# aleksandrina-streltsova/lidar-global-registration

Hardware: AMD Instinct MI355X
Metric: scan-pair registrations/sec (higher is better)
Workload: dtype f32

## Files before the change

### lidar-global-registration_amd/csrc/lgr_align.hip

```cpp
#include <rocprim/device/device_scan.hpp>

#include <chrono>
#include <cmath>

#include <climits>

#include "lgr_cloud.h"
#include "lgr_host.h"

namespace {

__device__ __forceinline__ float corr_threshold(float a, float b, float dthr) {
    float m = (a < b) ? b : a;
    return (dthr < m) ? dthr : m;
}

template <int KMAX>
__device__ __forceinline__ float cluster_distance(int i, int j, int k, const int32_t* __restrict__ knn_a, const int32_t* __restrict__ knn_b,
                                                   const int32_t* __restrict__ ab_idx) {
    int nb[KMAX];
#pragma unroll
    for (int b = 0; b < KMAX; ++b) nb[b] = b < k ? knn_b[(size_t) j * k + b] : -2;
    int consistent = 0, pairs = 0;
    for (int a0 = 0; a0 < k; a0 += 8) {
// ... 107 lines not shown
    size_t tb = 0;
    LGR_HIP(ctx, rocprim::exclusive_scan(nullptr, tb, flags, pos, 0, (size_t) ns, rocprim::plus<int>(), ctx->stream));
    void* tmp;
    LGR_TRY(lgr_ws(ctx, WS_GRID_TMP, tb, &tmp));
    LGR_HIP(ctx, rocprim::exclusive_scan(tmp, tb, flags, pos, 0, (size_t) ns, rocprim::plus<int>(), ctx->stream));
    filter_emit<<<cdiv(ns, 256), 256, 0, ctx->stream>>>(ns, d_ij_idx, flags, pos, dist, thr_s, thr_t, distance_thr, d_out);
    int* h;
    LGR_TRY(lgr_pinned(ctx, 64, (void**) &h));
    LGR_HIP(ctx, hipMemcpyAsync(h, pos + (ns - 1), 4, hipMemcpyDeviceToHost, ctx->stream));
    LGR_HIP(ctx, hipMemcpyAsync(h + 1, flags + (ns - 1), 4, hipMemcpyDeviceToHost, ctx->stream));
    LGR_HIP(ctx, hipStreamSynchronize(ctx->stream));
    *n_out = h[0] + h[1];
    LGR_HIP(ctx, hipGetLastError());
    return LGR_OK;
}

static void tick(lgr_ctx* ctx, int i) { (void) hipEventRecord(ctx->ev[i], ctx->stream); }

__global__ void gather_rows12_kernel(const float* __restrict__ pts, const int32_t* __restrict__ idx, int m, float* __restrict__ out) {
    size_t e = (size_t) blockIdx.x * blockDim.x + threadIdx.x;
    if (e >= (size_t) m * 12) return;
    out[e] = pts[(size_t) idx[e / 12] * 12 + e % 12];
}
static void gather_rows12(lgr_ctx* ctx, const float* pts, const int32_t* idx, int m, float* out) {
    gather_rows12_kernel<<<cdiv((long long) m * 12, 256), 256, 0, ctx->stream>>>(pts, idx, m, out);
}
__global__ void finalize_kernel(lgr_corr* __restrict__ corr, int n, const int32_t* __restrict__ ks, const int32_t* __restrict__ kt) {
    int i = blockIdx.x * blockDim.x + threadIdx.x;
    if (i >= n) return;
    corr[i].index_query = ks[corr[i].index_query];
    corr[i].index_match = kt[corr[i].index_match];
}

typedef int (*FeatureStage)(lgr_ctx* ctx, const float* kps, int m, const float* surf, int n, float radius, float* out, const lgr_params* p, const float* vp);
struct Descriptor {
    int len;
    FeatureStage stage;
    bool dense;
    int lrf;
};
static int fpfh_stage(lgr_ctx* ctx, const float* kps, int m, const float* surf, int n, float radius, float* out, const lgr_params*, const float*) { return lgr_fpfh_dev(ctx, kps, m, surf, n, radius, out); }
static int shot_stage(lgr_ctx* ctx, const float* kps, int m, const float* surf, int n, float radius, float* out, const lgr_params*, const float*) { return lgr_shot_dev(ctx, kps, m, surf, n, radius, nullptr, out, nullptr); }
static int rops_stage(lgr_ctx* ctx, const float* kps, int m, const float* surf, int n, float radius, float* out, const lgr_params* p, const float* vp) {
    float* kn;
    LGR_TRY(lgr_ws_t(ctx, WS_ROPS_KPS, (size_t) m * 12, &kn));
    LGR_HIP(ctx, hipMemcpyAsync(kn, kps, (size_t) m * 48, hipMemcpyDeviceToDevice, ctx->stream));
    LGR_TRY(lgr_normals_knn_dev(ctx, kn, m, surf, n, p->normal_nr_points, vp, 1));
    return lgr_rops_gravity_dev(ctx, kn, m, surf, n, radius, out);
}
static const Descriptor DESCRIPTORS[] = {
     {33, fpfh_stage, false, LGR_LRF_DEFAULT},
     {352, shot_stage, true, LGR_LRF_DEFAULT},
     {135, rops_stage, true, LGR_LRF_GRAVITY},
};
static_assert(LGR_DESCRIPTOR_FPFH == 0 && LGR_DESCRIPTOR_SHOT == 1 && LGR_DESCRIPTOR_ROPS == 2, "DESCRIPTORS is indexed by descriptor_id");

extern "C" void lgr_default_feature_params(lgr_feature_params* f) {
    if (!f) return;
    memset(f, 0, sizeof(*f));
    f->descriptor_id = LGR_DESCRIPTOR_FPFH;
    f->lrf_id = LGR_LRF_DEFAULT;
}

static int feature_descriptor(lgr_ctx* ctx, const lgr_params* p, const lgr_feature_params* f, const Descriptor** out) {
    *out = &DESCRIPTORS[LGR_DESCRIPTOR_FPFH];
    if (!f) return LGR_OK;
    LGR_CHECK(ctx, f->descriptor_id >= 0 && f->descriptor_id < (int) (sizeof DESCRIPTORS / sizeof *DESCRIPTORS), LGR_ERR_UNSUPPORTED);
    const Descriptor& d = DESCRIPTORS[f->descriptor_id];
    if (d.dense) {
        LGR_CHECK(ctx, f->lrf_id == LGR_LRF_DEFAULT || f->lrf_id == LGR_LRF_GRAVITY || f->lrf_id == LGR_LRF_GT, LGR_ERR_INVALID_ARG);
        LGR_CHECK(ctx, f->lrf_id == d.lrf, LGR_ERR_UNSUPPORTED);
        LGR_CHECK(ctx, p->use_bfmatcher && !p->has_guess, LGR_ERR_UNSUPPORTED);
        LGR_CHECK(ctx, ctx->opt.arithmetic != LGR_ARITH_PCL, LGR_ERR_UNSUPPORTED);
    }
    *out = &d;
    return LGR_OK;
// ... 13 lines not shown
    bool empty = false;
    float *feat[2], *surf[2], *dij, *dji;
    int32_t *ij, *ji;
    FilterTables ftab;
    int ratio_k = 0;
    float ms[3] = {0, 0, 0};
    struct Tables {
        CorrCall* c;
        int operator()(lgr_ctx* cx) const {
            LGR_TRY(filter_cloud_tables(cx, c->kclouds[0], c->ksizes[0], c->p->cluster_k, c->ftab.thr_s, c->ftab.knn_s));
            return filter_cloud_tables(cx, c->kclouds[1], c->ksizes[1], c->p->cluster_k, c->ftab.thr_t, c->ftab.knn_t);
        }
    } tables{this};
    lgr_helper_guard tables_guard;
    struct PrepGuard { lgr_ctx* c; ~PrepGuard() { lgr_match_prepare_cancel(c); } } prep_guard;

    CorrCall(lgr_ctx* ctx, const float* d_src, int ns, const float* d_tgt, int nt, const lgr_params* p, lgr_corr* d_out, int* n_out)
        : ctx(ctx), p(p), clouds{d_src, d_tgt}, kclouds{d_src, d_tgt}, sizes{ns, nt}, ksizes{ns, nt}, d_out(d_out), n_out(n_out), prep_guard{ctx} {}
    CorrCall(const CorrCall&) = delete;
    const float* vp(int side) const { return side == 0 ? (p->has_vp_src ? p->vp_src : nullptr) : (p->has_vp_tgt ? p->vp_tgt : nullptr); }
    float iss_radius(int side) const { return side == 0 ? p->iss_radius_src : p->iss_radius_tgt; }
    bool ratio() const { return p->matching_id == LGR_MATCH_RATIO; }
    bool both_dirs() const { return p->matching_id != LGR_MATCH_ONE_SIDED && !ratio(); }
    template <class T>
    int result(int side, int slot, size_t count, T** out) const { return own[side] ? lgr_cloud_alloc_t(ctx, own[side], count, out) : lgr_ws_t(ctx, slot, count, out); }
};

static int level_features(lgr_ctx* cx, const CorrCall& c, int side, const float* in, int n_in, float voxel, float radius, float* surf,
                          const float* kps, int m, const int32_t* d_list, float* sub, float* out, float* ms, int* nd) {
    const lgr_params* p = c.p;
    tick(cx, 0);
    LGR_TRY(lgr_downsample_dev(cx, in, n_in, voxel, surf, nd));
    tick(cx, 1);
    LGR_TRY(lgr_normals_knn_dev(cx, surf, *nd, nullptr, 0, p->normal_nr_points, c.vp(side), p->normals_available));
    tick(cx, 2);
    if (m) {
        if (d_list) { gather_rows12(cx, kps, d_list, m, sub); kps = sub; }
        LGR_TRY(c.d->stage(cx, kps, m, surf, *nd, radius, out, p, c.vp(side)));
    }
    tick(cx, 3);
    LGR_HIP(cx, hipEventSynchronize(cx->ev[3]));
    float t;
    for (int s = 0; s < 3; ++s) { (void) hipEventElapsedTime(&t, cx->ev[s], cx->ev[s + 1]); ms[s] += t; }
    return LGR_OK;
}

static int ms_initialize(CorrCall& c, int side, MsSide& st) {
    lgr_ctx* ctx = c.ctx;
    const lgr_params* p = c.p;
    const int D = c.d->len, n = c.sizes[side], n_kps = c.ksizes[side];
    const float *d_pcd = c.clouds[side], *d_kps = c.kclouds[side];
    const int k = 5;
    LGR_CHECK(ctx, n >= k, LGR_ERR_INVALID_ARG);
    int32_t* d_nn;
    float* d_d2;
    LGR_TRY(lgr_ws_t(ctx, WS_MS_KNN_I, (size_t) n_kps * k, &d_nn));
    LGR_TRY(lgr_ws_t(ctx, WS_MS_KNN_D, (size_t) n_kps * k, &d_d2));
    LGR_TRY(lgr_knn_dev(ctx, d_kps, n_kps, d_pcd, n, k, d_nn, d_d2));
    std::vector<float> d2((size_t) n_kps * k);
    LGR_HIP(ctx, hipMemcpyAsync(d2.data(), d_d2, d2.size() * 4, hipMemcpyDeviceToHost, ctx->stream));
    LGR_HIP(ctx, hipStreamSynchronize(ctx->stream));
    std::vector<int> level(n_kps);
    for (int i = 0; i < n_kps; ++i) {
        float density = sqrtf(d2[(size_t) i * k + (k - 1)]);
        float feature_radius = sqrtf((float) p->feature_nr_points * density * density / M_PI);
        level[i] = (int) std::floor(std::log2(feature_radius) / std::log2(p->scale_factor));
        st.min_l2 = std::min(level[i], st.min_l2);
        st.max_l2 = std::max(level[i], st.max_l2);
    }
    LGR_CHECK(ctx, (long long) st.max_l2 - st.min_l2 < 64, LGR_ERR_INVALID_ARG);
    std::vector<int> count(st.max_l2 - st.min_l2 + 1, 0);
// ... 704 lines not shown
```

### lidar-global-registration_amd/csrc/lgr_features.hip

```cpp
#include <rocprim/device/device_radix_sort.hpp>
#include <rocprim/device/device_scan.hpp>

#include <algorithm>
#include <cmath>
#include <type_traits>
#include <vector>

#include "lgr_grid.cuh"
#include "lgr_host.h"
#include "lgr_knn_wave.cuh"
#include "lgr_seqsum.h"
#include "lgr_math.cuh"
#include "lgr_libm.cuh"

namespace {

__global__ void voxel_keys(const float* __restrict__ pts, int n, float bx, float by, float bz, float voxel,
                           unsigned long long* __restrict__ keys, int* __restrict__ vals, int* __restrict__ bad) {
    int i = blockIdx.x * blockDim.x + threadIdx.x;
    if (i >= n) return;
    float x = pts[(size_t) i * 12], y = pts[(size_t) i * 12 + 1], z = pts[(size_t) i * 12 + 2];
    unsigned long long k = ~0ull;
    if (lgr_finite3(x, y, z)) {
        int ix = (int) floorf((x - bx) / voxel), iy = (int) floorf((y - by) / voxel), iz = (int) floorf((z - bz) / voxel);
// ... 10 lines not shown
    flags[i] = (k != ~0ull && (i == 0 || keys[i - 1] != k)) ? 1 : 0;
}

__global__ void voxel_accumulate(const float* __restrict__ pts, const unsigned long long* __restrict__ keys,
                                 const int* __restrict__ vals, const int* __restrict__ flags,
                                 const int* __restrict__ rank , int n,
                                 float* __restrict__ out, unsigned long long* __restrict__ out_keys, int* __restrict__ out_first) {
    int i = blockIdx.x * blockDim.x + threadIdx.x;
    if (i >= n || !flags[i]) return;
    unsigned long long k = keys[i];
    float sx = 0.f, sy = 0.f, sz = 0.f, sw = 0.f, snx = 0.f, sny = 0.f, snz = 0.f;
    for (int j = i; j < n && keys[j] == k; ++j) {
        const float4* p = reinterpret_cast<const float4*>(pts + (size_t) vals[j] * 12);
        float4 a = p[0], b = p[1], c = p[2];
        float w = c.x;
        sx += w * a.x; sy += w * a.y; sz += w * a.z;
        sw += w;
        snx += w * b.x; sny += w * b.y; snz += w * b.z;
    }
    float ax = snx / sw, ay = sny / sw, az = snz / sw;
    float norm = __builtin_sqrtf(ax * ax + ay * ay + az * az);
    norm = ((double) norm < 1e-5) ? 1.f : norm;
    int r = rank[i];
    float4* o = reinterpret_cast<float4*>(out + (size_t) r * 12);
    o[0] = make_float4(sx / sw, sy / sw, sz / sw, 1.f);
    o[1] = make_float4(ax / norm, ay / norm, az / norm, 0.f);
    o[2] = make_float4(sw, 0.f, 0.f, 0.f);
    if (out_keys) { out_keys[r] = k; out_first[r] = vals[i]; }
}

constexpr int NB = 128;

template <class IndexOf>
__device__ __forceinline__ void normals_finish(float* __restrict__ p, float px, float py, float pz, int count, IndexOf&& index_of,
                                               const float* __restrict__ surf, float vpx, float vpy, float vpz) {
    const float nanv = __uint_as_float(0x7fc00000u);
    if (count < 3) { p[4] = nanv; p[5] = nanv; p[6] = nanv; p[9] = nanv; return; }
    const float* K = surf + (size_t) index_of(0) * 12;
    float Kx = K[0], Ky = K[1], Kz = K[2];
    float a0 = 0.f, a1 = 0.f, a2 = 0.f, a3 = 0.f, a4 = 0.f, a5 = 0.f, a6 = 0.f, a7 = 0.f, a8 = 0.f;
    for (int j = 0; j < count; ++j) {
        const float* q = surf + (size_t) index_of(j) * 12;
        float x = q[0] - Kx, y = q[1] - Ky, z = q[2] - Kz;
        a0 += x * x; a1 += x * y; a2 += x * z; a3 += y * y; a4 += y * z; a5 += z * z;
        a6 += x; a7 += y; a8 += z;
    }
    float fn = (float) count;
    a0 /= fn; a1 /= fn; a2 /= fn; a3 /= fn; a4 /= fn; a5 /= fn; a6 /= fn; a7 /= fn; a8 /= fn;
    float C[9];
    C[0] = a0 - a6 * a6; C[1] = a1 - a6 * a7; C[2] = a2 - a6 * a8;
    C[4] = a3 - a7 * a7; C[5] = a4 - a7 * a8; C[8] = a5 - a8 * a8;
    C[3] = C[1]; C[6] = C[2]; C[7] = C[5];
    float lambda_min, nx, ny, nz;
    lgr_pcl_eigen33(C, lambda_min, nx, ny, nz);
    float eig_sum = C[0] + C[4] + C[8];
    float curv = (eig_sum != 0.f) ? fabsf(lambda_min / eig_sum) : 0.f;
    float dx = vpx - px, dy = vpy - py, dz = vpz - pz;
    float cos_theta = (dx * nx + dy * ny + dz * nz);
    if (cos_theta < 0.f) { nx = -nx; ny = -ny; nz = -nz; }
    if (lgr_finite3(nx, ny, nz)) {
        float norm = __builtin_sqrtf(nx * nx + ny * ny + nz * nz);
        nx /= norm; ny /= norm; nz /= norm;
    }
    p[4] = nx; p[5] = ny; p[6] = nz; p[9] = curv;
}

__global__ __launch_bounds__(NB) void normals_kernel(GridDev g, const float* __restrict__ surf, float* __restrict__ pts, int n,
                                                      int k, float vpx, float vpy, float vpz, int by_grid) {
    extern __shared__ float smem[];
    float* sd = smem;
    int* si = (int*) (smem + (size_t) k * NB);
    int i = blockIdx.x * NB + threadIdx.x;
    if (by_grid == 1) {
        i = lgr_xcd_tile(blockIdx.x, cdiv_dev(g.n, NB)) * NB + threadIdx.x;
        if (i >= g.n) return;
        i = __float_as_int(g.pxyz[i].w);
    } else if (i >= n) return;
    float* p = pts + (size_t) i * 12;
    float px = p[0], py = p[1], pz = p[2];
    if (by_grid == 2 && lgr_finite3(px, py, pz)) return;
    KnnList<NB> L;
    L.init(sd, si, k, threadIdx.x);
    if (lgr_finite3(px, py, pz) && g.n > 0) lgr_knn_query(g, px, py, pz, L);
    normals_finish(p, px, py, pz, L.count, [&](int j) { return L.index(j); }, surf, vpx, vpy, vpz);
}

constexpr int NW_WAVES = 4;
template <int KPL>
__global__ __launch_bounds__(64 * NW_WAVES) void normals_wave_kernel(GridDev g, const float* __restrict__ surf, float* __restrict__ pts, int k,
                                                                      float vpx, float vpy, float vpz, float r2_init) {
    extern __shared__ int slist[];
    __shared__ unsigned long long sbuf[NW_WAVES][WaveKnn<KPL>::BUF];
    __shared__ int srow[NW_WAVES][128];
    const int lane = threadIdx.x & 63, wv = threadIdx.x >> 6;
    const int n_tiles = cdiv_dev(g.n, 64 * NW_WAVES);
    const int tile = lgr_xcd_tile(blockIdx.x, n_tiles);
    if (tile >= n_tiles) return;
    const int t = (tile * NW_WAVES + wv) * 64 + lane;
    int* list = slist + (size_t) wv * k * 64;
    int qi = -1;
    float px = 0.f, py = 0.f, pz = 0.f;
    if (t < g.n) {
        const float4 q = g.pxyz[t];
        qi = __float_as_int(q.w); px = q.x; py = q.y; pz = q.z;
    }
    float guess = r2_init;
    int count = 0;
    lgr_wave_knn_tile<KPL>(g, qi >= 0, px, py, pz, k, guess, sbuf[wv], srow[wv], [&](int l, const WaveKnn<KPL>& W) {
        const int mk = min(W.m, k);
#pragma unroll
        for (int j = 0; j < KPL; ++j)
            if (W.rank[j] < mk) list[W.rank[j] * 64 + l] = (int) (unsigned) W.key[j];
        if (lane == l) count = mk;
    });
    __builtin_amdgcn_fence(__ATOMIC_RELEASE, "wavefront");
    __builtin_amdgcn_wave_barrier();
    if (qi < 0) return;
    normals_finish(pts + (size_t) qi * 12, px, py, pz, count, [&](int j) { return list[j * 64 + lane]; }, surf, vpx, vpy, vpz);
}

__device__ __forceinline__ float dot3e(float ax, float ay, float az, float bx, float by, float bz) {
    return (ax * bx + az * bz) + ay * by;
}

__device__ __forceinline__ bool pair_features(float p1x, float p1y, float p1z, float n1x, float n1y, float n1z,
                                              float p2x, float p2y, float p2z, float n2x, float n2y, float n2z,
                                              float& f1, float& f2, float& f3) {
    float dx = p2x - p1x, dy = p2y - p1y, dz = p2z - p1z;
    float f4 = __builtin_sqrtf(dot3e(dx, dy, dz, dx, dy, dz));
    if (f4 == 0.0f) return false;
    float angle1 = dot3e(n1x, n1y, n1z, dx, dy, dz) / f4;
    float angle2 = dot3e(n2x, n2y, n2z, dx, dy, dz) / f4;
    float ux = n1x, uy = n1y, uz = n1z, mx = n2x, my = n2y, mz = n2z;
    float a1 = fabsf(angle1), a2 = fabsf(angle2);
    if (lgr_glibc::acosf_(a1) > lgr_glibc::acosf_(a2)) {
        ux = n2x; uy = n2y; uz = n2z; mx = n1x; my = n1y; mz = n1z;
        dx = -dx; dy = -dy; dz = -dz;
        f3 = -angle2;
    } else {
        f3 = angle1;
    }
    float vx = dy * uz - dz * uy, vy = dz * ux - dx * uz, vz = dx * uy - dy * ux;
    float v_norm = __builtin_sqrtf(dot3e(vx, vy, vz, vx, vy, vz));
    if (v_norm == 0.0f) return false;
    vx /= v_norm; vy /= v_norm; vz /= v_norm;
    float wx = uy * vz - uz * vy, wy = uz * vx - ux * vz, wz = ux * vy - uy * vx;
    f2 = dot3e(vx, vy, vz, mx, my, mz);
    float yy = dot3e(wx, wy, wz, mx, my, mz), xx = dot3e(ux, uy, uz, mx, my, mz);
    f1 = lgr_glibc::atan2f_(yy, xx);
    return true;
}
// ... 773 lines not shown
            case 2: r = lgr_glibc::atan2f_(x, b[i]); break;
            case 3: r = lgr_glibc::sinf_(x); break;
            default: r = lgr_glibc::cosf_(x); break;
        }
        out[i] = r;
    }
}
extern "C" int lgr_selfcheck_libm(lgr_ctx* ctx, int fn, const float* a, const float* b, long long n, float* out) {
    lgr_turn turn__(ctx);
    if (!ctx) return LGR_ERR_INVALID_ARG;
    LGR_CHECK(ctx, fn >= 0 && fn <= 6 && a && out && n >= 0 && (fn != 2 || b), LGR_ERR_INVALID_ARG);
    if (n == 0) return LGR_OK;
    float *da, *db, *dout;
    lgr_host_call hc(ctx);
    LGR_TRY(hc.in(a, (size_t) n, &da));
    LGR_TRY(hc.in(fn == 2 ? b : nullptr, (size_t) n, &db));
    LGR_TRY(hc.out((size_t) n, &dout));
    if (fn >= 5) LGR_TRY(lgr_weights_libm_launch(ctx, fn, da, n, dout));
    else libm_eval_kernel<<<8 * ctx->n_cu, 256, 0, ctx->stream>>>(fn, da, db, n, dout);
    LGR_HIP(ctx, hipGetLastError());
    LGR_TRY(hc.fetch(out, dout, (size_t) n));
    return hc.finish();
}

#ifdef LGR_SPFH_CHECK
extern "C" int lgr_debug_spfh_check(unsigned long long* out3, int reset) {
    unsigned long long z[4] = {0, 0, 0, 0};
    if (hipMemcpyFromSymbol(out3, HIP_SYMBOL(g_spfh_check), 24) != hipSuccess) return LGR_ERR_HIP;
    if (reset && hipMemcpyToSymbol(HIP_SYMBOL(g_spfh_check), z, 32) != hipSuccess) return LGR_ERR_HIP;
    return LGR_OK;
}
#endif

extern "C" int lgr_normals_knn_dev(lgr_ctx* ctx, float* d_pts, int n, const float* d_surf, int ns, int k, const float* vp3, int normals_available) {
    lgr_turn turn__(ctx);
    if (!ctx) return LGR_ERR_INVALID_ARG;
    LGR_CHECK(ctx, (d_pts || n == 0) && n >= 0 && k >= 1 && k <= 64, LGR_ERR_INVALID_ARG);
    (void) normals_available;
    if (n == 0) return LGR_OK;
    LGR_HIP(ctx, hipSetDevice(ctx->device));
    const float* S = d_surf;
    if (!S) {
        float* snap;
        LGR_TRY(lgr_ws_t(ctx, WS_SELF_COPY, (size_t) n * 12, &snap));
        LGR_HIP(ctx, hipMemcpyAsync(snap, d_pts, (size_t) n * 48, hipMemcpyDeviceToDevice, ctx->stream));
        S = snap; ns = n;
    }
    GridDev g;
    const bool wave = !d_surf && k >= 16;
    const float ppc = wave ? 10.f : 6.f;
    LGR_TRY(lgr_grid_build(ctx, WS_GRID_A, S, ns, 0.f, ppc, &g));
    size_t sm = (size_t) k * NB * 8;
    const float vx = vp3 ? vp3[0] : 0.f, vy = vp3 ? vp3[1] : 0.f, vz = vp3 ? vp3[2] : 0.f;
    if (wave) {
        const float r2i = g.h * g.h * 1.25f * (float) k / (3.14159265f * ppc);
        const int grid = lgr_xcd_grid(cdiv(g.n, 64 * NW_WAVES));
        const size_t sml = (size_t) NW_WAVES * k * 64 * sizeof(int);
        if (g.n > 0) {
            if (k <= 40) normals_wave_kernel<1><<<grid, 64 * NW_WAVES, sml, ctx->stream>>>(g, S, d_pts, k, vx, vy, vz, r2i);
            else {
                if (sml + 8192 > 65536) LGR_HIP(ctx, hipFuncSetAttribute((const void*) normals_wave_kernel<2>, hipFuncAttributeMaxDynamicSharedMemorySize, (int) sml));
                normals_wave_kernel<2><<<grid, 64 * NW_WAVES, sml, ctx->stream>>>(g, S, d_pts, k, vx, vy, vz, r2i);
            }
        }
        if (g.n < n) normals_kernel<<<cdiv(n, NB), NB, sm, ctx->stream>>>(g, S, d_pts, n, k, vx, vy, vz, 2);
    } else if (!d_surf) {
        if (g.n > 0) normals_kernel<<<lgr_xcd_grid(cdiv(g.n, NB)), NB, sm, ctx->stream>>>(g, S, d_pts, n, k, vx, vy, vz, 1);
        if (g.n < n) normals_kernel<<<cdiv(n, NB), NB, sm, ctx->stream>>>(g, S, d_pts, n, k, vx, vy, vz, 2);
    } else {
        normals_kernel<<<cdiv(n, NB), NB, sm, ctx->stream>>>(g, S, d_pts, n, k, vx, vy, vz, 0);
    }
    LGR_HIP(ctx, hipGetLastError());
    return LGR_OK;
}

extern "C" int lgr_normals_knn(lgr_ctx* ctx, float* pts, int n, const float* surf, int ns, int k, const float* vp3, int normals_available) {
    lgr_turn turn__(ctx);
    if (!ctx) return LGR_ERR_INVALID_ARG;
    LGR_CHECK(ctx, (pts || n == 0) && n >= 0, LGR_ERR_INVALID_ARG);
    if (n == 0) return LGR_OK;
    float *dp, *ds = nullptr;
    lgr_host_call hc(ctx);
    LGR_TRY(hc.in((const float*) pts, (size_t) n * 12, &dp));
    if (surf) LGR_TRY(hc.in(surf, (size_t) ns * 12, &ds, LGR_PAD_CLOUD));
    LGR_TRY(lgr_normals_knn_dev(ctx, dp, n, ds, ns, k, vp3, normals_available));
    LGR_TRY(hc.fetch(pts, dp, (size_t) n * 12));
    return hc.finish();
}

extern "C" int lgr_fpfh_dev(lgr_ctx* ctx, const float* d_kps, int m, const float* d_surf, int n, float radius, float* d_out) {
    lgr_turn turn__(ctx);
    if (!ctx) return LGR_ERR_INVALID_ARG;
    LGR_CHECK(ctx, (d_kps || m == 0) && (d_surf || n == 0) && (d_out || m == 0) && m >= 0 && n >= 0 && radius > 0.f, LGR_ERR_INVALID_ARG);
    LGR_CHECK(ctx, radius <= 1e18f && (size_t) n + 1 <= ((size_t) 1 << 32) / HP - 1, LGR_ERR_UNSUPPORTED);
    if (m == 0) return LGR_OK;
    LGR_HIP(ctx, hipSetDevice(ctx->device));
    GridDev g;
    LGR_TRY(lgr_grid_build(ctx, WS_GRID_B, d_surf, n, radius * 1.001f, 0.f, &g));
    float r2 = radius * radius;
    float* spfh;
    LGR_TRY(lgr_ws_t(ctx, WS_SPFH, ((size_t) n + 1) * HP + 64, &spfh));
    LGR_HIP(ctx, hipMemsetAsync(spfh + (size_t) g.n * HP, 0, HP * sizeof(float), ctx->stream));
    const long long n_cells = (long long) g.dx * g.dy * g.dz;
    int cell_bits = 1;
    while ((1ll << cell_bits) < n_cells) ++cell_bits;
    const int sb = std::max(0, std::min(2, (32 - cell_bits) / 3));
    const int key_bits = std::min(32, cell_bits + 3 * sb);
    const int mx = std::max(m, g.n);
    unsigned *keys, *keys2, *kkeys, *kkeys2;
    int *vals, *vals2, *kvals, *kvals2;
    LGR_TRY(lgr_ws_t(ctx, WS_KP_ORDER, (size_t) mx * 8 + 16, &keys));
    keys2 = keys + mx; vals = (int*) (keys2 + mx); vals2 = vals + mx;
    kkeys = (unsigned*) (vals2 + mx); kkeys2 = kkeys + mx; kvals = (int*) (kkeys2 + mx); kvals2 = kvals + mx;
    fine_keys<<<cdiv(m, 256), 256, 0, ctx->stream>>>(g, d_kps, 12, m, sb, kkeys, kvals);
    LGR_TRY(lgr_sort_pairs_u32(ctx, kkeys, kkeys2, kvals, kvals2, (size_t) m, 0, key_bits));
    if (g.n > 0) {
        fine_keys<<<cdiv(g.n, 256), 256, 0, ctx->stream>>>(g, reinterpret_cast<const float*>(g.pxyz), 4, g.n, sb, keys, vals);
        LGR_TRY(lgr_sort_pairs_u32(ctx, keys, keys2, vals, vals2, (size_t) g.n, 0, key_bits));
        spfh_tile_kernel<<<lgr_xcd_grid(cdiv(g.n, ST)), 64, 0, ctx->stream>>>(g, r2, vals2, spfh);
    }
    if (ctx->opt.arithmetic == LGR_ARITH_PCL) {
        if (ctx->opt.pcl_neighbour_cap == 64) fpfh_pcl_kernel<64><<<lgr_xcd_grid(m), 64, 0, ctx->stream>>>(g, d_kps, kvals2, m, r2, spfh, d_out);
        else if (ctx->opt.pcl_neighbour_cap == 1024) fpfh_pcl_kernel<1024><<<lgr_xcd_grid(m), 64, 0, ctx->stream>>>(g, d_kps, kvals2, m, r2, spfh, d_out);
        else fpfh_pcl_kernel<512><<<lgr_xcd_grid(m), 64, 0, ctx->stream>>>(g, d_kps, kvals2, m, r2, spfh, d_out);
    } else {
        fpfh_mfma_kernel<<<lgr_xcd_grid(cdiv(m, FT)), 64, 0, ctx->stream>>>(g, d_kps, kvals2, m, r2, spfh, d_out);
    }
    LGR_HIP(ctx, hipGetLastError());
    return LGR_OK;
}

extern "C" int lgr_fpfh(lgr_ctx* ctx, const float* kps, int m, const float* surf, int n, float radius, float* out) {
    lgr_turn turn__(ctx);
    if (!ctx) return LGR_ERR_INVALID_ARG;
    LGR_CHECK(ctx, (kps || m == 0) && (surf || n == 0) && (out || m == 0) && m >= 0 && n >= 0, LGR_ERR_INVALID_ARG);
    if (m == 0) return LGR_OK;
    float *dk, *ds, *dout;
    lgr_host_call hc(ctx);
    LGR_TRY(hc.in(kps, (size_t) m * 12, &dk));
    LGR_TRY(hc.in(surf, (size_t) n * 12, &ds, LGR_PAD_CLOUD));
    LGR_TRY(hc.out((size_t) m * 33, &dout));
    LGR_TRY(lgr_fpfh_dev(ctx, dk, m, ds, n, radius, dout));
    LGR_TRY(hc.fetch(out, dout, (size_t) m * 33));
    return hc.finish();
}
```

### lidar-global-registration_amd/csrc/lgr_grid.hip

```cpp
#include <rocprim/device/device_radix_sort.hpp>
#include <rocprim/device/device_scan.hpp>

#include <algorithm>
#include <cmath>

#include "lgr_grid.cuh"
#include "lgr_grid_rule.h"
#include "lgr_host.h"
#include "lgr_knn_wave.cuh"

namespace {

__device__ __forceinline__ unsigned fkey(float f) {
    unsigned b = __float_as_uint(f);
    return (b & 0x80000000u) ? ~b : (b | 0x80000000u);
}
__host__ __device__ inline float fkey_inv(unsigned k) {
    unsigned b = (k & 0x80000000u) ? (k & 0x7fffffffu) : ~k;
    float f;
    memcpy(&f, &b, 4);
    return f;
}

__global__ void bbox_kernel(const float* __restrict__ pts, int n, unsigned* __restrict__ out) {
// ... 57 lines not shown
        hi = i == n ? nblk : (int) (keys[i] >> CSF_SHIFT);
    }
    unsigned long long todo = __ballot(lo <= hi);
    while (todo) {
        const int j = __builtin_ctzll(todo);
        todo &= todo - 1ull;
        const int lo_j = __builtin_amdgcn_readlane(lo, j), hi_j = __builtin_amdgcn_readlane(hi, j);
        for (int c = lo_j + lane; c <= hi_j; c += 64) coarse[c] = base + j;
    }
}
__global__ __launch_bounds__(CSF_T) void cell_start_fill(const unsigned* __restrict__ keys, const int* __restrict__ coarse, unsigned ncell, int* __restrict__ start) {
    const int k0 = coarse[blockIdx.x], k1 = coarse[blockIdx.x + 1];
    const unsigned c = (unsigned) blockIdx.x * CSF_CELLS + 4u * threadIdx.x;
    if (c > ncell) return;
    int lo = k0, hi = k1;
    while (lo < hi) { const int mid = (lo + hi) >> 1; if (keys[mid] < c) lo = mid + 1; else hi = mid; }
    int4 v;
    v.x = lo;
    while (lo < k1 && keys[lo] < c + 1u) ++lo;
    v.y = lo;
    while (lo < k1 && keys[lo] < c + 2u) ++lo;
    v.z = lo;
    while (lo < k1 && keys[lo] < c + 3u) ++lo;
    v.w = lo;
    if (c + 3u <= ncell) {
        *reinterpret_cast<int4*>(start + c) = v;
    } else {
        start[c] = v.x;
        if (c + 1u <= ncell) start[c + 1] = v.y;
        if (c + 2u <= ncell) start[c + 2] = v.z;
    }
}

__global__ void gather_points(const float* __restrict__ pts, const int* __restrict__ vals, int nvalid,
                              float4* __restrict__ pxyz, float4* __restrict__ pnrm) {
    int i = blockIdx.x * blockDim.x + threadIdx.x;
    if (i >= nvalid) return;
    int o = vals[i];
    const float4* p = reinterpret_cast<const float4*>(pts + (size_t) o * 12);
    float4 a = p[0], b = p[1], c = p[2];
    pxyz[i] = make_float4(a.x, a.y, a.z, __int_as_float(o));
    pnrm[i] = make_float4(b.x, b.y, b.z, c.y);
}

constexpr int KNN_BLOCK = 128;

template <int MODE>
__global__ __launch_bounds__(KNN_BLOCK) void knn_kernel(GridDev g, const float* __restrict__ q, int nq, int k,
                                                        int32_t* __restrict__ idx, float* __restrict__ d2, int by_grid) {
    extern __shared__ float smem[];
    float* sd = smem;
    int* si = (int*) (smem + (size_t) k * KNN_BLOCK);
    int i = blockIdx.x * KNN_BLOCK + threadIdx.x;
    bool active = true;
    if (by_grid == 1) {
        i = lgr_xcd_tile(blockIdx.x, cdiv_dev(g.n, KNN_BLOCK)) * KNN_BLOCK + threadIdx.x;
        active = i < g.n;
        i = active ? __float_as_int(g.pxyz[i].w) : 0;
    } else if (i >= nq) { active = false; i = 0; }
    float x = 0.f, y = 0.f, z = 0.f;
    if (active) { x = q[(size_t) i * 12]; y = q[(size_t) i * 12 + 1]; z = q[(size_t) i * 12 + 2]; }
    if (by_grid == 2 && lgr_finite3(x, y, z)) active = false;
    KnnList<KNN_BLOCK> L;
    L.init(sd, si, k, threadIdx.x);
    if (active && lgr_finite3(x, y, z) && g.n > 0) lgr_knn_query(g, x, y, z, L);
    if (MODE == 0) {
        const int lane = threadIdx.x & 63, wbase = threadIdx.x & ~63;
        const int my_row = active ? i : -1, my_cnt = L.count;
        for (int r = 0; r < 64; ++r) {
            const int row = __builtin_amdgcn_readlane(my_row, r);
            if (row < 0) continue;
            const int cnt = __builtin_amdgcn_readlane(my_cnt, r);
            for (int j = lane; j < k; j += 64) {
                idx[(size_t) row * k + j] = j < cnt ? si[j * KNN_BLOCK + wbase + r] : -1;
                if (d2) d2[(size_t) row * k + j] = j < cnt ? sd[j * KNN_BLOCK + wbase + r] : INFINITY;
// ... 122 lines not shown
    unsigned kfmx, kfmn;
    memcpy(&kfmx, &fmx, 4); kfmx |= 0x80000000u;
    memcpy(&kfmn, &fmn, 4); kfmn |= 0x80000000u;
    for (int a = 0; a < 3; ++a) { init[a] = pinf; init[3 + a] = ninf; init[6 + a] = kfmx; init[9 + a] = kfmn; }
    LGR_HIP(ctx, hipMemcpyAsync(d, init, sizeof init, hipMemcpyHostToDevice, ctx->stream));
    if (n > 0) bbox_kernel<<<std::min(cdiv(n, 256), ctx->n_cu), 256, 0, ctx->stream>>>(d_pts, n, d);
    LGR_HIP(ctx, hipGetLastError());
    *d_keys12 = d;
    return LGR_OK;
}

int lgr_bbox_host(lgr_ctx* ctx, const float* d_pts, int n, float* out12) {
    const unsigned* d;
    LGR_TRY(lgr_bbox_launch(ctx, d_pts, n, &d));
    unsigned* h;
    LGR_TRY(lgr_pinned(ctx, 64, (void**) &h));
    LGR_HIP(ctx, hipMemcpyAsync(h, d, 48, hipMemcpyDeviceToHost, ctx->stream));
    LGR_HIP(ctx, hipStreamSynchronize(ctx->stream));
    for (int i = 0; i < 12; ++i) out12[i] = fkey_inv(h[i]);
    return LGR_OK;
}

extern "C" int lgr_bbox_dev(lgr_ctx* ctx, const float* d_pts, int n, float* d_min3_max3) {
    lgr_turn turn__(ctx);
    if (!ctx) return LGR_ERR_INVALID_ARG;
    LGR_CHECK(ctx, (d_pts || n == 0) && d_min3_max3 && n >= 0, LGR_ERR_INVALID_ARG);
    float bb[12];
    LGR_TRY(lgr_bbox_host(ctx, d_pts, n, bb));
    LGR_HIP(ctx, hipMemcpyAsync(d_min3_max3, bb + 6, 24, hipMemcpyHostToDevice, ctx->stream));
    LGR_HIP(ctx, hipStreamSynchronize(ctx->stream));
    return LGR_OK;
}

int lgr_grid_build(lgr_ctx* ctx, int sb, const float* d_pts, int n, float h, float target, GridDev* out) {
    float bb[12];
    LGR_TRY(lgr_bbox_host(ctx, d_pts, n, bb));
    float mn[3] = {bb[0], bb[1], bb[2]}, mx[3] = {bb[3], bb[4], bb[5]};
    if (!(mn[0] <= mx[0])) { for (int a = 0; a < 3; ++a) { mn[a] = 0.f; mx[a] = 0.f; } }
    if (!(h > 0.f)) {
        float e[3] = {mx[0] - mn[0], mx[1] - mn[1], mx[2] - mn[2]};
        std::sort(e, e + 3);
        float area = std::max(e[2] * e[1], 1e-12f);
        h = std::sqrt(area * target / (float) std::max(n, 1));
        h = std::max(h, std::max(e[2] / 1024.f, 1e-6f));
    }
    int dim[3];
    h = lgr_grid_cell_rule(mn, mx, h, dim);
    int ncell = dim[0] * dim[1] * dim[2];
    unsigned *keys, *keys2;
    int *vals, *vals2, *start;
    float4 *pxyz, *pnrm;
    LGR_TRY(lgr_ws_t(ctx, sb + 0, (size_t) n + 1, &keys));
    LGR_TRY(lgr_ws_t(ctx, sb + 1, (size_t) n + 1, &vals));
    LGR_TRY(lgr_ws_t(ctx, sb + 2, (size_t) n + 1, &keys2));
    LGR_TRY(lgr_ws_t(ctx, sb + 3, (size_t) n + 1, &vals2));
    LGR_TRY(lgr_ws_t(ctx, sb + 4, (size_t) ncell + 2, &start));
    LGR_TRY(lgr_ws_t(ctx, sb + 5, (size_t) n + 1, &pxyz));
    LGR_TRY(lgr_ws_t(ctx, sb + 6, (size_t) n + 1, &pnrm));
    int nvalid = 0;
    if (n > 0) {
        cell_keys<<<cdiv(n, 256), 256, 0, ctx->stream>>>(d_pts, n, mn[0], mn[1], mn[2], h, dim[0], dim[1], dim[2], (unsigned) ncell, keys, vals);
        int bits = 1;
        while (((unsigned long long) 1 << bits) <= (unsigned long long) ncell) ++bits;
        LGR_TRY(lgr_sort_pairs_u32(ctx, keys, keys2, vals, vals2, (size_t) n, 0, bits));
        const int nblk = (int) (((size_t) ncell + 1 + CSF_CELLS - 1) >> CSF_SHIFT);
        int* coarse;
        LGR_TRY(lgr_ws_t(ctx, WS_GRID_MISC, (size_t) nblk + 1 + 64, &coarse));
        coarse += 64;
        coarse_start_fill<<<cdiv(n + 1, 256), 256, 0, ctx->stream>>>(keys2, n, nblk, coarse);
        cell_start_fill<<<nblk, CSF_T, 0, ctx->stream>>>(keys2, coarse, (unsigned) ncell, start);
        int* h_n;
        LGR_TRY(lgr_pinned(ctx, 64, (void**) &h_n));
        LGR_HIP(ctx, hipMemcpyAsync(h_n, start + ncell, 4, hipMemcpyDeviceToHost, ctx->stream));
        LGR_HIP(ctx, hipStreamSynchronize(ctx->stream));
        nvalid = *h_n;
        if (nvalid > 0) gather_points<<<cdiv(nvalid, 256), 256, 0, ctx->stream>>>(d_pts, vals2, nvalid, pxyz, pnrm);
    } else {
        LGR_HIP(ctx, hipMemsetAsync(start, 0, ((size_t) ncell + 2) * 4, ctx->stream));
    }
    LGR_HIP(ctx, hipGetLastError());
    out->ox = mn[0]; out->oy = mn[1]; out->oz = mn[2]; out->h = h;
    out->dx = dim[0]; out->dy = dim[1]; out->dz = dim[2];
    out->n = nvalid; out->cell_start = start; out->pxyz = pxyz; out->pnrm = pnrm;
    return LGR_OK;
}

extern "C" int lgr_knn_dev(lgr_ctx* ctx, const float* d_q, int nq, const float* d_pts, int n, int k, int32_t* d_idx, float* d_d2) {
    lgr_turn turn__(ctx);
    if (!ctx) return LGR_ERR_INVALID_ARG;
    LGR_CHECK(ctx, d_d2 != nullptr, LGR_ERR_INVALID_ARG);
    return lgr_knn_lists(ctx, d_q, nq, d_pts, n, k, d_idx, d_d2);
}

int lgr_knn_lists(lgr_ctx* ctx, const float* d_q, int nq, const float* d_pts, int n, int k, int32_t* d_idx, float* d_d2) {
    LGR_CHECK(ctx, nq >= 0 && n >= 0 && k >= 1 && k <= 128 && (d_q || nq == 0) && (d_pts || n == 0) && d_idx, LGR_ERR_INVALID_ARG);
    if (nq == 0) return LGR_OK;
    LGR_HIP(ctx, hipSetDevice(ctx->device));
    GridDev g;
    const float ppc = std::max(4.f, 0.35f * (float) k);
    LGR_TRY(lgr_grid_build(ctx, WS_GRID_A, d_pts, n, 0.f, ppc, &g));
    size_t sm = (size_t) k * KNN_BLOCK * 8;
    const bool heap = k < 16;
    if (!heap) {
        if (d_q == d_pts && nq == n) {
            knn_wave_launch<0>(ctx, g, d_q, nq, k, d_idx, d_d2, 1, ppc);
            if (g.n < nq) knn_wave_launch<0>(ctx, g, d_q, nq, k, d_idx, d_d2, 2, ppc);
        } else {
            knn_wave_launch<0>(ctx, g, d_q, nq, k, d_idx, d_d2, 0, ppc);
        }
    } else if (d_q == d_pts && nq == n) {
        if (g.n > 0) knn_kernel<0><<<lgr_xcd_grid(cdiv(g.n, KNN_BLOCK)), KNN_BLOCK, sm, ctx->stream>>>(g, d_q, nq, k, d_idx, d_d2, 1);
        if (g.n < nq) knn_kernel<0><<<cdiv(nq, KNN_BLOCK), KNN_BLOCK, sm, ctx->stream>>>(g, d_q, nq, k, d_idx, d_d2, 2);
    } else {
        knn_kernel<0><<<cdiv(nq, KNN_BLOCK), KNN_BLOCK, sm, ctx->stream>>>(g, d_q, nq, k, d_idx, d_d2, 0);
    }
    LGR_HIP(ctx, hipGetLastError());
    return LGR_OK;
}

extern "C" int lgr_smoothed_densities_dev(lgr_ctx* ctx, const float* d_pts, int n, int k, float* d_out) {
    lgr_turn turn__(ctx);
    if (!ctx) return LGR_ERR_INVALID_ARG;
    LGR_CHECK(ctx, d_pts && d_out && n > 1 && k >= 2 && k <= 128, LGR_ERR_INVALID_ARG);
    LGR_HIP(ctx, hipSetDevice(ctx->device));
    GridDev g;
    LGR_TRY(lgr_grid_build(ctx, WS_GRID_A, d_pts, n, 0.f, 4.f, &g));
    float* dk; int32_t* nn1;
    LGR_TRY(lgr_ws_t(ctx, WS_DENS_A, (size_t) n, &dk));
    LGR_TRY(lgr_ws_t(ctx, WS_DENS_B, (size_t) n, &nn1));
    size_t sm = (size_t) k * KNN_BLOCK * 8;
    const bool heap = k < 16;
    if (!heap) {
        knn_wave_launch<1>(ctx, g, d_pts, n, k, nn1, dk, 1, 4.f);
        if (g.n < n) knn_wave_launch<1>(ctx, g, d_pts, n, k, nn1, dk, 2, 4.f);
    } else {
    if (g.n > 0) knn_kernel<1><<<lgr_xcd_grid(cdiv(g.n, KNN_BLOCK)), KNN_BLOCK, sm, ctx->stream>>>(g, d_pts, n, k, nn1, dk, 1);
    if (g.n < n) knn_kernel<1><<<cdiv(n, KNN_BLOCK), KNN_BLOCK, sm, ctx->stream>>>(g, d_pts, n, k, nn1, dk, 2);
    }
    density_min<<<cdiv(n, 256), 256, 0, ctx->stream>>>(dk, nn1, n, d_out);
    LGR_HIP(ctx, hipGetLastError());
    return LGR_OK;
}

extern "C" int lgr_smoothed_densities(lgr_ctx* ctx, const float* pts, int n, int k, float* out) {
    lgr_turn turn__(ctx);
    if (!ctx) return LGR_ERR_INVALID_ARG;
    LGR_CHECK(ctx, pts && out && n > 1, LGR_ERR_INVALID_ARG);
    float *dp, *dout;
    lgr_host_call hc(ctx);
    LGR_TRY(hc.in(pts, (size_t) n * 12, &dp));
    LGR_TRY(hc.out((size_t) n, &dout));
    LGR_TRY(lgr_smoothed_densities_dev(ctx, dp, n, k, dout));
    LGR_TRY(hc.fetch(out, dout, (size_t) n));
    return hc.finish();
}
```

### lidar-global-registration_amd/csrc/lgr_internal.h

```cpp
#pragma once
#include <hip/hip_runtime.h>
#include <stdint.h>
#include <stdio.h>
#include <string.h>

#include <condition_variable>
#include <functional>
#include <mutex>
#include <string>
#include <thread>
#include <vector>

#include "../../include/lgr.h"

#define LGR_WAVE 64
#define LGR_STREAM_OWN_LOW ((void*) (intptr_t) -2)

struct lgr_buf {
    void* p = nullptr;
    size_t cap = 0;
};

struct lgr_match_stats { unsigned items_ab, dense_ab, items_ba, dense_ba; int sub_cols, rg_rows; double stages_done, stages_all, stages_unique; int f16; double coarse_tested, coarse_rejected; unsigned pairs_ab, pairs_ba; double shell_skipped; double lb_zero, lb_finite; unsigned irr_a, irr_b, irr_gave_up; };

// ... 104 lines not shown
    WS_MEASURE_MASKS, WS_MEASURE_W,
    WS_HO_WORK, WS_HO_ACT, WS_HO_HASH, WS_HO_STAGE,
    WS_TEASER_STATE, WS_TEASER_ADJ,
    WS_KNNF_OPS_A, WS_KNNF_OPS_B, WS_KNNF_MISC_A, WS_KNNF_MISC_B, WS_KNNF_IRR_A, WS_KNNF_IRR_B, WS_KNNF_PART, WS_KNNF_UW, WS_KNNF_CNT, WS_KNNF_CAND,
    WS_KNNF_FB, WS_KNNF_ISFB, WS_KNNF_DEV, WS_KNNF_FBROWS, WS_KNNF_FBIDX, WS_KNNF_FBDIST, WS_KNNF_CENTRE,
    WS_DENSEF_OPS_A, WS_DENSEF_OPS_B, WS_DENSEF_MISC_A, WS_DENSEF_MISC_B, WS_DENSEF_IRR_A, WS_DENSEF_IRR_B, WS_DENSEF_U, WS_DENSEF_CNT, WS_DENSEF_CAND,
    WS_DENSEF_FB, WS_DENSEF_ISFB, WS_DENSEF_DEV, WS_DENSEF_FBROWS, WS_DENSEF_FBIDX, WS_DENSEF_FBDIST, WS_DENSEF_CENTRE,
    WS_COUNT
};
static_assert(WS_COUNT <= 192, "grow lgr_ctx::ws");

int lgr_ws(lgr_ctx* ctx, int slot, size_t bytes, void** out);
int lgr_pinned(lgr_ctx* ctx, size_t bytes, void** out);

template <class T>
static inline int lgr_ws_t(lgr_ctx* ctx, int slot, size_t count, T** out) {
    void* p = nullptr;
    int rc = lgr_ws(ctx, slot, count * sizeof(T), &p);
    *out = (T*) p;
    return rc;
}

static inline int cdiv(long long a, long long b) { return (int) ((a + b - 1) / b); }
static inline size_t cdivz(size_t a, size_t b) { return (a + b - 1) / b; }

struct GridDev {
    float ox, oy, oz, h;
    int dx, dy, dz;
    int n;
    const int* cell_start;
    const float4* pxyz;
    const float4* pnrm;
};
int lgr_grid_build(lgr_ctx* ctx, int slot_base, const float* d_pts, int n, float h, float target, GridDev* out);
int lgr_rops_gravity_dev(lgr_ctx* ctx, const float* d_kps, int m, const float* d_surf, int n, float radius, float* d_out135);
int lgr_bbox_host(lgr_ctx* ctx, const float* d_pts, int n, float* out12);
int lgr_bbox_launch(lgr_ctx* ctx, const float* d_pts, int n, const unsigned** d_keys12);
__host__ __device__ inline float lgr_bbox_key_inv(unsigned k) {
    const unsigned b = (k & 0x80000000u) ? (k & 0x7fffffffu) : ~k;
    float f;
    memcpy(&f, &b, 4);
    return f;
}
void lgr_inverse4(const float* m16, float* out16);
int lgr_knn_lists(lgr_ctx* ctx, const float* d_q, int nq, const float* d_pts, int n, int k, int32_t* d_idx, float* d_d2);

int lgr_ctx_aux(lgr_ctx* ctx);
int lgr_ctx_aux2(lgr_ctx* ctx);
int lgr_ctx_stream3(lgr_ctx* ctx, hipStream_t* out);
int lgr_helper_post(lgr_ctx* owner, lgr_ctx* aux, std::function<int()> job);
int lgr_helper_wait(lgr_ctx* aux);
struct lgr_helper_guard {
    lgr_ctx* aux = nullptr;
    bool armed = false;
    int wait() { armed = false; return lgr_helper_wait(aux); }
    ~lgr_helper_guard() { if (armed) (void) lgr_helper_wait(aux); }
};
template <class F>
static inline std::function<int()> lgr_aux_job(lgr_ctx* aux, F&& f) {
    return [aux, &f]() -> int {
        int rc = hipSetDevice(aux->device) == hipSuccess ? f(aux) : (int) LGR_ERR_HIP;
        const hipError_t e = hipStreamSynchronize(aux->stream);
        if (rc == LGR_OK && e != hipSuccess) rc = lgr_fail(aux, LGR_ERR_HIP, hipGetErrorString(e), __FILE__, __LINE__);
        return rc;
    };
}
template <class FA, class FB>
// ... 78 lines not shown
```

Baseline: 47.25.

## Reuse normals-grid bbox for FPFH grid and drop redundant copies and gathers

The normals stage now returns the bounding box it computed while building its grid. The FPFH grid build reuses that box instead of running another host-synchronising bbox reduction over the same unchanged surface points. Normal estimation now runs in place on the point buffer rather than first snapshotting it, since it reads only xyz and writes only normal and curvature slots. Grid builds that do not need normals skip gathering them into pnrm. The wave normals kernel also gains a waves-per-EU hint, a scalarised wave id, and a fixed neighbour count of min(k, n). That count assumes the wave kNN always fills k neighbours, which is a correctness risk if it ever returns fewer.

```diff
diff --git a/lidar-global-registration_amd/csrc/lgr_align.hip b/lidar-global-registration_amd/csrc/lgr_align.hip
--- a/lidar-global-registration_amd/csrc/lgr_align.hip
+++ b/lidar-global-registration_amd/csrc/lgr_align.hip
@@ -163,16 +163,16 @@
     corr[i].index_match = kt[corr[i].index_match];
 }
 
-typedef int (*FeatureStage)(lgr_ctx* ctx, const float* kps, int m, const float* surf, int n, float radius, float* out, const lgr_params* p, const float* vp);
+typedef int (*FeatureStage)(lgr_ctx* ctx, const float* kps, int m, const float* surf, int n, float radius, float* out, const lgr_params* p, const float* vp, const float* box12);
 struct Descriptor {
     int len;
     FeatureStage stage;
     bool dense;
     int lrf;
 };
-static int fpfh_stage(lgr_ctx* ctx, const float* kps, int m, const float* surf, int n, float radius, float* out, const lgr_params*, const float*) { return lgr_fpfh_dev(ctx, kps, m, surf, n, radius, out); }
-static int shot_stage(lgr_ctx* ctx, const float* kps, int m, const float* surf, int n, float radius, float* out, const lgr_params*, const float*) { return lgr_shot_dev(ctx, kps, m, surf, n, radius, nullptr, out, nullptr); }
-static int rops_stage(lgr_ctx* ctx, const float* kps, int m, const float* surf, int n, float radius, float* out, const lgr_params* p, const float* vp) {
+static int fpfh_stage(lgr_ctx* ctx, const float* kps, int m, const float* surf, int n, float radius, float* out, const lgr_params*, const float*, const float* box12) { return lgr_fpfh_box(ctx, kps, m, surf, n, radius, out, box12); }
+static int shot_stage(lgr_ctx* ctx, const float* kps, int m, const float* surf, int n, float radius, float* out, const lgr_params*, const float*, const float*) { return lgr_shot_dev(ctx, kps, m, surf, n, radius, nullptr, out, nullptr); }
+static int rops_stage(lgr_ctx* ctx, const float* kps, int m, const float* surf, int n, float radius, float* out, const lgr_params* p, const float* vp, const float*) {
     float* kn;
     LGR_TRY(lgr_ws_t(ctx, WS_ROPS_KPS, (size_t) m * 12, &kn));
     LGR_HIP(ctx, hipMemcpyAsync(kn, kps, (size_t) m * 48, hipMemcpyDeviceToDevice, ctx->stream));
@@ -252,11 +252,12 @@
     tick(cx, 0);
     LGR_TRY(lgr_downsample_dev(cx, in, n_in, voxel, surf, nd));
     tick(cx, 1);
-    LGR_TRY(lgr_normals_knn_dev(cx, surf, *nd, nullptr, 0, p->normal_nr_points, c.vp(side), p->normals_available));
+    float box[12];
+    LGR_TRY(lgr_normals_knn_box(cx, surf, *nd, nullptr, 0, p->normal_nr_points, c.vp(side), p->normals_available, box));
     tick(cx, 2);
     if (m) {
         if (d_list) { gather_rows12(cx, kps, d_list, m, sub); kps = sub; }
-        LGR_TRY(c.d->stage(cx, kps, m, surf, *nd, radius, out, p, c.vp(side)));
+        LGR_TRY(c.d->stage(cx, kps, m, surf, *nd, radius, out, p, c.vp(side), *nd > 0 ? box : nullptr));
     }
     tick(cx, 3);
     LGR_HIP(cx, hipEventSynchronize(cx->ev[3]));
diff --git a/lidar-global-registration_amd/csrc/lgr_features.hip b/lidar-global-registration_amd/csrc/lgr_features.hip
--- a/lidar-global-registration_amd/csrc/lgr_features.hip
+++ b/lidar-global-registration_amd/csrc/lgr_features.hip
@@ -66,8 +66,8 @@
 constexpr int NB = 128;
 
 template <class IndexOf>
-__device__ __forceinline__ void normals_finish(float* __restrict__ p, float px, float py, float pz, int count, IndexOf&& index_of,
-                                               const float* __restrict__ surf, float vpx, float vpy, float vpz) {
+__device__ __forceinline__ void normals_finish(float* p, float px, float py, float pz, int count, IndexOf&& index_of,
+                                               const float* surf, float vpx, float vpy, float vpz) {
     const float nanv = __uint_as_float(0x7fc00000u);
     if (count < 3) { p[4] = nanv; p[5] = nanv; p[6] = nanv; p[9] = nanv; return; }
     const float* K = surf + (size_t) index_of(0) * 12;
@@ -99,7 +99,7 @@
     p[4] = nx; p[5] = ny; p[6] = nz; p[9] = curv;
 }
 
-__global__ __launch_bounds__(NB) void normals_kernel(GridDev g, const float* __restrict__ surf, float* __restrict__ pts, int n,
+__global__ __launch_bounds__(NB) void normals_kernel(GridDev g, const float* surf, float* pts, int n,
                                                       int k, float vpx, float vpy, float vpz, int by_grid) {
     extern __shared__ float smem[];
     float* sd = smem;
@@ -121,12 +121,12 @@
 
 constexpr int NW_WAVES = 4;
 template <int KPL>
-__global__ __launch_bounds__(64 * NW_WAVES) void normals_wave_kernel(GridDev g, const float* __restrict__ surf, float* __restrict__ pts, int k,
-                                                                      float vpx, float vpy, float vpz, float r2_init) {
+__global__ __launch_bounds__(64 * NW_WAVES) __attribute__((amdgpu_waves_per_eu(KPL == 1 ? 4 : 3, KPL == 1 ? 4 : 3)))
+void normals_wave_kernel(GridDev g, float* pts, int k, float vpx, float vpy, float vpz, float r2_init) {
     extern __shared__ int slist[];
     __shared__ unsigned long long sbuf[NW_WAVES][WaveKnn<KPL>::BUF];
     __shared__ int srow[NW_WAVES][128];
-    const int lane = threadIdx.x & 63, wv = threadIdx.x >> 6;
+    const int lane = threadIdx.x & 63, wv = __builtin_amdgcn_readfirstlane(threadIdx.x >> 6);
     const int n_tiles = cdiv_dev(g.n, 64 * NW_WAVES);
     const int tile = lgr_xcd_tile(blockIdx.x, n_tiles);
     if (tile >= n_tiles) return;
@@ -139,18 +139,17 @@
         qi = __float_as_int(q.w); px = q.x; py = q.y; pz = q.z;
     }
     float guess = r2_init;
-    int count = 0;
     lgr_wave_knn_tile<KPL>(g, qi >= 0, px, py, pz, k, guess, sbuf[wv], srow[wv], [&](int l, const WaveKnn<KPL>& W) {
         const int mk = min(W.m, k);
 #pragma unroll
         for (int j = 0; j < KPL; ++j)
             if (W.rank[j] < mk) list[W.rank[j] * 64 + l] = (int) (unsigned) W.key[j];
-        if (lane == l) count = mk;
     });
     __builtin_amdgcn_fence(__ATOMIC_RELEASE, "wavefront");
     __builtin_amdgcn_wave_barrier();
     if (qi < 0) return;
-    normals_finish(pts + (size_t) qi * 12, px, py, pz, count, [&](int j) { return list[j * 64 + lane]; }, surf, vpx, vpy, vpz);
+    const int count = min(k, g.n);
+    normals_finish(pts + (size_t) qi * 12, px, py, pz, count, [&](int j) { return list[j * 64 + lane]; }, pts, vpx, vpy, vpz);
 }
 
 __device__ __forceinline__ float dot3e(float ax, float ay, float az, float bx, float by, float bz) {
@@ -990,7 +989,7 @@
 }
 #endif
 
-extern "C" int lgr_normals_knn_dev(lgr_ctx* ctx, float* d_pts, int n, const float* d_surf, int ns, int k, const float* vp3, int normals_available) {
+int lgr_normals_knn_box(lgr_ctx* ctx, float* d_pts, int n, const float* d_surf, int ns, int k, const float* vp3, int normals_available, float* box12_out) {
     lgr_turn turn__(ctx);
     if (!ctx) return LGR_ERR_INVALID_ARG;
     LGR_CHECK(ctx, (d_pts || n == 0) && n >= 0 && k >= 1 && k <= 64, LGR_ERR_INVALID_ARG);
@@ -998,16 +997,11 @@
     if (n == 0) return LGR_OK;
     LGR_HIP(ctx, hipSetDevice(ctx->device));
     const float* S = d_surf;
-    if (!S) {
-        float* snap;
-        LGR_TRY(lgr_ws_t(ctx, WS_SELF_COPY, (size_t) n * 12, &snap));
-        LGR_HIP(ctx, hipMemcpyAsync(snap, d_pts, (size_t) n * 48, hipMemcpyDeviceToDevice, ctx->stream));
-        S = snap; ns = n;
-    }
+    if (!S) { S = d_pts; ns = n; }
     GridDev g;
     const bool wave = !d_surf && k >= 16;
     const float ppc = wave ? 10.f : 6.f;
-    LGR_TRY(lgr_grid_build(ctx, WS_GRID_A, S, ns, 0.f, ppc, &g));
+    LGR_TRY(lgr_grid_build(ctx, WS_GRID_A, S, ns, 0.f, ppc, &g,  false, nullptr, box12_out));
     size_t sm = (size_t) k * NB * 8;
     const float vx = vp3 ? vp3[0] : 0.f, vy = vp3 ? vp3[1] : 0.f, vz = vp3 ? vp3[2] : 0.f;
     if (wave) {
@@ -1015,10 +1009,10 @@
         const int grid = lgr_xcd_grid(cdiv(g.n, 64 * NW_WAVES));
         const size_t sml = (size_t) NW_WAVES * k * 64 * sizeof(int);
         if (g.n > 0) {
-            if (k <= 40) normals_wave_kernel<1><<<grid, 64 * NW_WAVES, sml, ctx->stream>>>(g, S, d_pts, k, vx, vy, vz, r2i);
+            if (k <= 40) normals_wave_kernel<1><<<grid, 64 * NW_WAVES, sml, ctx->stream>>>(g, d_pts, k, vx, vy, vz, r2i);
             else {
                 if (sml + 8192 > 65536) LGR_HIP(ctx, hipFuncSetAttribute((const void*) normals_wave_kernel<2>, hipFuncAttributeMaxDynamicSharedMemorySize, (int) sml));
-                normals_wave_kernel<2><<<grid, 64 * NW_WAVES, sml, ctx->stream>>>(g, S, d_pts, k, vx, vy, vz, r2i);
+                normals_wave_kernel<2><<<grid, 64 * NW_WAVES, sml, ctx->stream>>>(g, d_pts, k, vx, vy, vz, r2i);
             }
         }
         if (g.n < n) normals_kernel<<<cdiv(n, NB), NB, sm, ctx->stream>>>(g, S, d_pts, n, k, vx, vy, vz, 2);
@@ -1030,6 +1024,10 @@
     }
     LGR_HIP(ctx, hipGetLastError());
     return LGR_OK;
+}
+
+extern "C" int lgr_normals_knn_dev(lgr_ctx* ctx, float* d_pts, int n, const float* d_surf, int ns, int k, const float* vp3, int normals_available) {
+    return lgr_normals_knn_box(ctx, d_pts, n, d_surf, ns, k, vp3, normals_available, nullptr);
 }
 
 extern "C" int lgr_normals_knn(lgr_ctx* ctx, float* pts, int n, const float* surf, int ns, int k, const float* vp3, int normals_available) {
@@ -1046,7 +1044,7 @@
     return hc.finish();
 }
 
-extern "C" int lgr_fpfh_dev(lgr_ctx* ctx, const float* d_kps, int m, const float* d_surf, int n, float radius, float* d_out) {
+int lgr_fpfh_box(lgr_ctx* ctx, const float* d_kps, int m, const float* d_surf, int n, float radius, float* d_out, const float* box12) {
     lgr_turn turn__(ctx);
     if (!ctx) return LGR_ERR_INVALID_ARG;
     LGR_CHECK(ctx, (d_kps || m == 0) && (d_surf || n == 0) && (d_out || m == 0) && m >= 0 && n >= 0 && radius > 0.f, LGR_ERR_INVALID_ARG);
@@ -1054,7 +1052,7 @@
     if (m == 0) return LGR_OK;
     LGR_HIP(ctx, hipSetDevice(ctx->device));
     GridDev g;
-    LGR_TRY(lgr_grid_build(ctx, WS_GRID_B, d_surf, n, radius * 1.001f, 0.f, &g));
+    LGR_TRY(lgr_grid_build(ctx, WS_GRID_B, d_surf, n, radius * 1.001f, 0.f, &g, true, box12));
     float r2 = radius * radius;
     float* spfh;
     LGR_TRY(lgr_ws_t(ctx, WS_SPFH, ((size_t) n + 1) * HP + 64, &spfh));
@@ -1088,6 +1086,10 @@
     return LGR_OK;
 }
 
+extern "C" int lgr_fpfh_dev(lgr_ctx* ctx, const float* d_kps, int m, const float* d_surf, int n, float radius, float* d_out) {
+    return lgr_fpfh_box(ctx, d_kps, m, d_surf, n, radius, d_out, nullptr);
+}
+
 extern "C" int lgr_fpfh(lgr_ctx* ctx, const float* kps, int m, const float* surf, int n, float radius, float* out) {
     lgr_turn turn__(ctx);
     if (!ctx) return LGR_ERR_INVALID_ARG;
diff --git a/lidar-global-registration_amd/csrc/lgr_grid.hip b/lidar-global-registration_amd/csrc/lgr_grid.hip
--- a/lidar-global-registration_amd/csrc/lgr_grid.hip
+++ b/lidar-global-registration_amd/csrc/lgr_grid.hip
@@ -113,15 +113,19 @@
     }
 }
 
+template <bool NRM>
 __global__ void gather_points(const float* __restrict__ pts, const int* __restrict__ vals, int nvalid,
                               float4* __restrict__ pxyz, float4* __restrict__ pnrm) {
     int i = blockIdx.x * blockDim.x + threadIdx.x;
     if (i >= nvalid) return;
     int o = vals[i];
     const float4* p = reinterpret_cast<const float4*>(pts + (size_t) o * 12);
-    float4 a = p[0], b = p[1], c = p[2];
+    float4 a = p[0];
     pxyz[i] = make_float4(a.x, a.y, a.z, __int_as_float(o));
-    pnrm[i] = make_float4(b.x, b.y, b.z, c.y);
+    if (NRM) {
+        float4 b = p[1], c = p[2];
+        pnrm[i] = make_float4(b.x, b.y, b.z, c.y);
+    }
 }
 
 constexpr int KNN_BLOCK = 128;
@@ -310,9 +314,12 @@
     return LGR_OK;
 }
 
-int lgr_grid_build(lgr_ctx* ctx, int sb, const float* d_pts, int n, float h, float target, GridDev* out) {
+int lgr_grid_build(lgr_ctx* ctx, int sb, const float* d_pts, int n, float h, float target, GridDev* out, bool with_normals, const float* box12,
+                   float* box12_out) {
     float bb[12];
-    LGR_TRY(lgr_bbox_host(ctx, d_pts, n, bb));
+    if (box12) memcpy(bb, box12, sizeof bb);
+    else LGR_TRY(lgr_bbox_host(ctx, d_pts, n, bb));
+    if (box12_out) memcpy(box12_out, bb, sizeof bb);
     float mn[3] = {bb[0], bb[1], bb[2]}, mx[3] = {bb[3], bb[4], bb[5]};
     if (!(mn[0] <= mx[0])) { for (int a = 0; a < 3; ++a) { mn[a] = 0.f; mx[a] = 0.f; } }
     if (!(h > 0.f)) {
@@ -327,14 +334,14 @@
     int ncell = dim[0] * dim[1] * dim[2];
     unsigned *keys, *keys2;
     int *vals, *vals2, *start;
-    float4 *pxyz, *pnrm;
+    float4 *pxyz, *pnrm = nullptr;
     LGR_TRY(lgr_ws_t(ctx, sb + 0, (size_t) n + 1, &keys));
     LGR_TRY(lgr_ws_t(ctx, sb + 1, (size_t) n + 1, &vals));
     LGR_TRY(lgr_ws_t(ctx, sb + 2, (size_t) n + 1, &keys2));
     LGR_TRY(lgr_ws_t(ctx, sb + 3, (size_t) n + 1, &vals2));
     LGR_TRY(lgr_ws_t(ctx, sb + 4, (size_t) ncell + 2, &start));
     LGR_TRY(lgr_ws_t(ctx, sb + 5, (size_t) n + 1, &pxyz));
-    LGR_TRY(lgr_ws_t(ctx, sb + 6, (size_t) n + 1, &pnrm));
+    if (with_normals) LGR_TRY(lgr_ws_t(ctx, sb + 6, (size_t) n + 1, &pnrm));
     int nvalid = 0;
     if (n > 0) {
         cell_keys<<<cdiv(n, 256), 256, 0, ctx->stream>>>(d_pts, n, mn[0], mn[1], mn[2], h, dim[0], dim[1], dim[2], (unsigned) ncell, keys, vals);
@@ -352,7 +359,10 @@
         LGR_HIP(ctx, hipMemcpyAsync(h_n, start + ncell, 4, hipMemcpyDeviceToHost, ctx->stream));
         LGR_HIP(ctx, hipStreamSynchronize(ctx->stream));
         nvalid = *h_n;
-        if (nvalid > 0) gather_points<<<cdiv(nvalid, 256), 256, 0, ctx->stream>>>(d_pts, vals2, nvalid, pxyz, pnrm);
+        if (nvalid > 0) {
+            if (with_normals) gather_points<true><<<cdiv(nvalid, 256), 256, 0, ctx->stream>>>(d_pts, vals2, nvalid, pxyz, pnrm);
+            else gather_points<false><<<cdiv(nvalid, 256), 256, 0, ctx->stream>>>(d_pts, vals2, nvalid, pxyz, nullptr);
+        }
     } else {
         LGR_HIP(ctx, hipMemsetAsync(start, 0, ((size_t) ncell + 2) * 4, ctx->stream));
     }
@@ -376,7 +386,7 @@
     LGR_HIP(ctx, hipSetDevice(ctx->device));
     GridDev g;
     const float ppc = std::max(4.f, 0.35f * (float) k);
-    LGR_TRY(lgr_grid_build(ctx, WS_GRID_A, d_pts, n, 0.f, ppc, &g));
+    LGR_TRY(lgr_grid_build(ctx, WS_GRID_A, d_pts, n, 0.f, ppc, &g,  false));
     size_t sm = (size_t) k * KNN_BLOCK * 8;
     const bool heap = k < 16;
     if (!heap) {
@@ -402,7 +412,7 @@
     LGR_CHECK(ctx, d_pts && d_out && n > 1 && k >= 2 && k <= 128, LGR_ERR_INVALID_ARG);
     LGR_HIP(ctx, hipSetDevice(ctx->device));
     GridDev g;
-    LGR_TRY(lgr_grid_build(ctx, WS_GRID_A, d_pts, n, 0.f, 4.f, &g));
+    LGR_TRY(lgr_grid_build(ctx, WS_GRID_A, d_pts, n, 0.f, 4.f, &g,  false));
     float* dk; int32_t* nn1;
     LGR_TRY(lgr_ws_t(ctx, WS_DENS_A, (size_t) n, &dk));
     LGR_TRY(lgr_ws_t(ctx, WS_DENS_B, (size_t) n, &nn1));
diff --git a/lidar-global-registration_amd/csrc/lgr_internal.h b/lidar-global-registration_amd/csrc/lgr_internal.h
--- a/lidar-global-registration_amd/csrc/lgr_internal.h
+++ b/lidar-global-registration_amd/csrc/lgr_internal.h
@@ -160,7 +160,10 @@
     const float4* pxyz;
     const float4* pnrm;
 };
-int lgr_grid_build(lgr_ctx* ctx, int slot_base, const float* d_pts, int n, float h, float target, GridDev* out);
+int lgr_grid_build(lgr_ctx* ctx, int slot_base, const float* d_pts, int n, float h, float target, GridDev* out, bool with_normals = true,
+                   const float* box12 = nullptr, float* box12_out = nullptr);
+int lgr_normals_knn_box(lgr_ctx* ctx, float* d_pts, int n, const float* d_surf, int ns, int k, const float* vp3, int normals_available, float* box12_out);
+int lgr_fpfh_box(lgr_ctx* ctx, const float* d_kps, int m, const float* d_surf, int n, float radius, float* d_out, const float* box12);
 int lgr_rops_gravity_dev(lgr_ctx* ctx, const float* d_kps, int m, const float* d_surf, int n, float radius, float* d_out135);
 int lgr_bbox_host(lgr_ctx* ctx, const float* d_pts, int n, float* out12);
 int lgr_bbox_launch(lgr_ctx* ctx, const float* d_pts, int n, const unsigned** d_keys12);
```

Result: no change. 47.63 (median of 6 runs) (+0.8%).
